# TThuraya/multimodal-PL

Hardware: AMD Instinct MI355X
Metric: train voxels/sec at 96^3 patch, 1/2/4/8 MI355X; fwd+bwd step ms (higher is better)
Workload: dtype bf16; 1 GPU; unet3D_baseline([1,2,2,2,2],16,weight_std) fwd+EDiceLoss_partial+bwd+SGD; model=unet3D_baseline-16, global_batch=2, seq_len=884736, parallelism=dp1, world_size_seen=1, force_buckets=False

## Files before the change

multimodal-pl_amd/csrc/common.h:

```cpp
#pragma once
#include <hip/hip_runtime.h>
#include <hip/hip_bf16.h>
#include <stdint.h>
#include <algorithm>
#include <string>
#include <type_traits>

#include "../../include/u3d.h"

namespace u3d {

void set_error(const std::string& msg);
int fail(int code, const char* fmt, ...);
int check_launch(const char* what);

enum Opt : int {
  OPT_IGEMM_BN,
  OPT_IGEMM_NS,
  OPT_IGEMM_TARGET,
  OPT_IGEMM_AUTO,
  OPT_CONVG_CO32,
  OPT_CONVG_PERSIST,
  OPT_CONVG_BW8,
  OPT_RING_KR,
  OPT_RING_WGS,
  OPT_RING_SC,
  OPT_SMALL_WGS,
  OPT_GN_MAXBLK,
  OPT_HEAD_TR,
  OPT_STEM1,
  OPT_UP_BWD_BLK,
  OPT_WGRAD_BD,
  OPT_WB_WGS,
  OPT_WR_TILE16,
  OPT_WR_WGS,
  OPT_WB_S2CO64,
  OPT_IGEMM_BM,
  OPT_WSTD_ROW,
  OPT_UP_QUAD,
  OPT_LOSS_PAIR,
  OPT_HEAD_NB,
  OPT_HEAD_GN_NB,
  OPT_STEM_MFMA,
  OPT_WB_S2BD,
  OPT_COUNT
};
int opt(Opt o);

#define U3D_REQUIRE(cond, ...)                                  \
  do {                                                          \
    if (!(cond)) return ::u3d::fail(U3D_EINVAL, __VA_ARGS__);   \
  } while (0)
#define U3D_HIP(expr)                                                               \
  do {                                                                              \
    hipError_t e_ = (expr);                                                         \
    if (e_ != hipSuccess)                                                           \
      return ::u3d::fail(U3D_EHIP, "%s: %s", #expr, hipGetErrorString(e_));         \
  } while (0)

template <int I, int N, typename F>
__device__ __forceinline__ void static_for(F&& f) {
  if constexpr (I < N) {
    f(std::integral_constant<int, I>{});
    static_for<I + 1, N>(f);
  }
}

typedef uint16_t bf16;

__device__ __forceinline__ float to_f(float v) { return v; }
__device__ __forceinline__ float to_f(bf16 v) { return __uint_as_float(((uint32_t)v) << 16); }

template <typename T> __device__ __forceinline__ T from_f(float v);
template <> __device__ __forceinline__ float from_f<float>(float v) { return v; }
template <> __device__ __forceinline__ bf16 from_f<bf16>(float v) {
  __hip_bfloat16 h = __float2bfloat16(v);
  return *reinterpret_cast<bf16*>(&h);
}

typedef __attribute__((ext_vector_type(4))) float f32x4;
typedef __attribute__((ext_vector_type(16))) float f32x16;
typedef __attribute__((ext_vector_type(8))) short s16x8;
typedef __attribute__((ext_vector_type(4))) uint32_t u32x4;

typedef __attribute__((ext_vector_type(2))) float f32x2;
typedef __attribute__((ext_vector_type(2))) __bf16 bf16x2_t;
typedef __attribute__((ext_vector_type(2))) short s16x2;

__device__ __forceinline__ uint32_t pack_bf16x2(float a, float b) {
  return __builtin_bit_cast(uint32_t, __builtin_convertvector((f32x2){a, b}, bf16x2_t));
}
__device__ __forceinline__ uint32_t relu_bf16x2(uint32_t u) {
  return __builtin_bit_cast(uint32_t, __builtin_elementwise_max(__builtin_bit_cast(s16x2, u), (s16x2){0, 0}));
}

template <int CTRL>
__device__ __forceinline__ float dpp_mov(float x) {
// ... 199 lines not shown
  *reinterpret_cast<u32x4*>(p) = r;
}

template <typename T, int N>
__device__ __forceinline__ void loadv(const T* p, float (&v)[N]) {
  if constexpr (N * sizeof(T) == 16) {
    load16<T>(p, v);
  } else {
#pragma unroll
    for (int i = 0; i < N; ++i) v[i] = to_f(p[i]);
  }
}
template <typename T, int N>
__device__ __forceinline__ void storev(T* p, const float (&v)[N]) {
  if constexpr (N * sizeof(T) == 16) {
    store16<T>(p, v);
  } else {
#pragma unroll
    for (int i = 0; i < N; ++i) p[i] = from_f<T>(v[i]);
  }
}

__device__ __forceinline__ u32x4 gn_relu8(u32x4 v, const f32x2 (&sc)[4], const f32x2 (&sh)[4]) {
  u32x4 o;
#pragma unroll
  for (int e = 0; e < 4; ++e) {
    const float f0 = fmaf(__uint_as_float(v[e] << 16), sc[e][0], sh[e][0]);
    const float f1 = fmaf(__uint_as_float(v[e] & 0xffff0000u), sc[e][1], sh[e][1]);
    o[e] = relu_bf16x2(pack_bf16x2(f0, f1));
  }
  return o;
}

__device__ __forceinline__ void gn_coef8(const float* __restrict__ st, const float* __restrict__ gamma,
                                         const float* __restrict__ beta, int groups, int cin, int n, int c0,
                                         f32x2 (&sc)[4], f32x2 (&sh)[4]) {
  const int cpg = cin / groups;
  const auto srs = __builtin_amdgcn_make_buffer_rsrc((void*)st, 0, 0x7FFFFFFF, 0x00020000);
  const auto grs = __builtin_amdgcn_make_buffer_rsrc((void*)gamma, 0, 0x7FFFFFFF, 0x00020000);
  const auto brs = __builtin_amdgcn_make_buffer_rsrc((void*)beta, 0, 0x7FFFFFFF, 0x00020000);
  asm volatile("" : "+v"(c0));
#pragma unroll
  for (int e = 0; e < 8; ++e) {
    const int c = min(c0 + e, cin - 1), gg = c / cpg;
    const int so = (n * groups + gg) * 8;
    const float mean = __builtin_bit_cast(float, __builtin_amdgcn_raw_buffer_load_b32(srs, so, 0, 0));
    const float rstd = __builtin_bit_cast(float, __builtin_amdgcn_raw_buffer_load_b32(srs, so + 4, 0, 0));
    const float s = rstd * __builtin_bit_cast(float, __builtin_amdgcn_raw_buffer_load_b32(grs, c * 4, 0, 0));
    sc[e >> 1][e & 1] = s;
    sh[e >> 1][e & 1] = __builtin_bit_cast(float, __builtin_amdgcn_raw_buffer_load_b32(brs, c * 4, 0, 0)) - mean * s;
  }
}

__device__ __forceinline__ float wave_sum(float v) {
#pragma unroll
  for (int o = 32; o > 0; o >>= 1) v += __shfl_xor(v, o, 64);
  return v;
}
__device__ __forceinline__ double wave_sum(double v) {
#pragma unroll
  for (int o = 32; o > 0; o >>= 1) v += __shfl_xor(v, o, 64);
  return v;
}

struct TileSplit {
  int tx, ty, split;
};
__device__ __forceinline__ TileSplit xcd_tile_split(int L, int gx, int gy, int total) {
  const int nt = gx * gy;
  const int q = total >> 3, rr = total & 7, xcd = L & 7, loc = L >> 3;
  const int N = (xcd < rr ? xcd * (q + 1) : rr * (q + 1) + (xcd - rr) * q) + loc;
  const int tile = N % nt;
  return TileSplit{tile % gx, tile / gx, N / nt};
}
__device__ __forceinline__ TileSplit xcd_tile_split() {
  return xcd_tile_split(blockIdx.x + gridDim.x * (blockIdx.y + gridDim.y * blockIdx.z), gridDim.x, gridDim.y,
                        gridDim.x * gridDim.y * gridDim.z);
}

__host__ __device__ inline int cdiv(long long a, long long b) { return (int)((a + b - 1) / b); }
__host__ __device__ inline int round_up(int a, int b) { return (a + b - 1) / b * b; }
inline bool fits_buffer_offsets(long long bytes) { return bytes < (1LL << 31) - 64; }

}
```

multimodal-pl_amd/csrc/conv.hip:

```cpp
#include <algorithm>
#include <cstdlib>

#include "common.h"

namespace u3d {

constexpr int BK = 32;
constexpr int NTHR = 256;

struct Geom {
  int cin, cout, cin_p, cout_p;
  int id, ih, iw;
  int od, oh, ow;
  int qd, qh, qw;
  int so, pod, poh, pow_;
  int si;
  int ntaps;
  int gn_groups;
  int nsamp, nsplit, kps;
  int mtiles, ntiles;
  float* slab;
  int tap_w[27];
  signed char tap_d[27], tap_h[27], tap_x[27];
};

template <typename T> struct MfmaTraits;
template <> struct MfmaTraits<bf16> {
  static constexpr int NCH = BK * 2 / 16;
  __device__ static int swz(int r, int c) { return c ^ ((r >> 2) & 3); }
};
template <> struct MfmaTraits<float> {
  static constexpr int NCH = BK * 4 / 16;
  __device__ static int swz(int r, int c) { return c ^ (r & 7); }
};

typedef __attribute__((ext_vector_type(8))) __bf16 bf16x8;

template <typename T, int TM, int TN>
__device__ __forceinline__ void mfma_step(const char* As, const char* Bs, int arow0, int brow0, int lane,
                                          f32x16 (&acc)[TM][TN]) {
  using TR = MfmaTraits<T>;
  constexpr int ROWB = BK * sizeof(T);
  const int r = lane & 31, h = lane >> 5;
  if constexpr (sizeof(T) == 2) {
#pragma unroll
    for (int s = 0; s < 2; ++s) {
      bf16x8 a[TM], b[TN];
#pragma unroll
      for (int tm = 0; tm < TM; ++tm) {
        int row = arow0 + tm * 32 + r;
        a[tm] = *reinterpret_cast<const bf16x8*>(As + row * ROWB + TR::swz(row, 2 * s + h) * 16);
      }
#pragma unroll
      for (int tn = 0; tn < TN; ++tn) {
        int row = brow0 + tn * 32 + r;
        b[tn] = *reinterpret_cast<const bf16x8*>(Bs + row * ROWB + TR::swz(row, 2 * s + h) * 16);
      }
#pragma unroll
      for (int tm = 0; tm < TM; ++tm)
#pragma unroll
        for (int tn = 0; tn < TN; ++tn)
          acc[tm][tn] = __builtin_amdgcn_mfma_f32_32x32x16_bf16(a[tm], b[tn], acc[tm][tn], 0, 0, 0);
    }
  } else {
#pragma unroll
    for (int j = 0; j < 4; ++j) {
      f32x4 a[TM], b[TN];
#pragma unroll
      for (int tm = 0; tm < TM; ++tm) {
        int row = arow0 + tm * 32 + r;
        a[tm] = *reinterpret_cast<const f32x4*>(As + row * ROWB + TR::swz(row, 4 * h + j) * 16);
      }
#pragma unroll
      for (int tn = 0; tn < TN; ++tn) {
// ... 149 lines not shown
  const int kk0 = split * g.kps, kk1 = min(nk, kk0 + g.kps);
  __syncthreads();
  if (kk0 < kk1) {
    gload(kk0);
    swrite(kk0, 0);
  }
  __syncthreads();
  for (int kk = kk0; kk < kk1; ++kk) {
    const int cur = (kk - kk0) & 1;
    if (kk + 1 < kk1) gload(kk + 1);
    mfma_step<T, TM, TN>(As(cur), Bs(cur), arow0, brow0, lane, acc);
    if (kk + 1 < kk1) swrite(kk + 1, cur ^ 1);
    __syncthreads();
  }

  const int r = lane & 31, h = lane >> 5;
  const long long out_n = (long long)n * g.od * g.oh * g.ow;
#pragma unroll
  for (int tn = 0; tn < TN; ++tn) {
    const int co = bn0 + brow0 + tn * 32 + r;
    if (co >= g.cout) continue;
    const float bv = bias ? bias[co] : 0.f;
#pragma unroll
    for (int tm = 0; tm < TM; ++tm) {
#pragma unroll
      for (int i = 0; i < 16; ++i) {
        const int q = bm0 + arow0 + tm * 32 + (i & 3) + 8 * (i >> 2) + 4 * h;
        if (q >= Mq) continue;
        if (g.nsplit > 1) {
          g.slab[(((long long)split * g.nsamp + n) * Mq + q) * g.cout + co] = acc[tm][tn][i];
          continue;
        }
        long long ov;
        if (g.so == 1) {
          ov = q;
        } else {
          int qw_ = q % g.qw, t = q / g.qw;
          int qh_ = t % g.qh, qd_ = t / g.qh;
          ov = ((long long)(qd_ * g.so + g.pod) * g.oh + (qh_ * g.so + g.poh)) * g.ow + (qw_ * g.so + g.pow_);
        }
        const long long off = (out_n + ov) * g.cout + co;
        float v = acc[tm][tn][i] + bv;
        if (res) v += to_f(res[off]);
        y[off] = from_f<TO>(v);
      }
    }
  }
}

template <int KC>
__device__ __forceinline__ int kswz(int r, int c) {
  if constexpr (KC == 4) return c ^ ((r >> 2) & 3);
  else return c ^ ((r >> 1) & 7);
}

template <typename TO, int BM, int BN, int WM, int WN, int KC>
__global__ __launch_bounds__(NTHR) void igemm_bf16_kernel(const bf16* __restrict__ x, const bf16* __restrict__ wpk,
                                                          TO* __restrict__ y, const bf16* __restrict__ res,
                                                          const float* __restrict__ bias,
                                                          const float* __restrict__ gstat,
                                                          const float* __restrict__ gamma,
                                                          const float* __restrict__ beta, Geom g) {
#ifndef U3D_IGEMM_D4
#define U3D_IGEMM_D4 3
#endif
#ifndef U3D_IGEMM_D8
#define U3D_IGEMM_D8 2
#endif
  constexpr int NCH = KC, ROWB = KC * 16, BKC = KC * 8, D = KC == 4 ? U3D_IGEMM_D4 : U3D_IGEMM_D8;
  constexpr int A_LOADS = BM * NCH / NTHR;
  constexpr int B_CH = BN * NCH;
  constexpr int B_LOADS = (B_CH + NTHR - 1) / NTHR;
  constexpr int TM = BM / WM / 32, TN = BN / WN / 32;
  static_assert(A_LOADS >= 1 && WM * WN == 4, "tile");

  __shared__ __attribute__((aligned(16))) char smem[2 * (BM + BN) * ROWB + 2 * 256 * 4 + 27 * 24];
  float* gsc = reinterpret_cast<float*>(smem + 2 * (BM + BN) * ROWB);
  float* gsh = gsc + 256;
  int* taps = reinterpret_cast<int*>(gsh + 256);
  int* tdhw = taps + 27 * 2;
  if (threadIdx.x < g.ntaps) {
    const int td = g.tap_d[threadIdx.x], th = g.tap_h[threadIdx.x], tx = g.tap_x[threadIdx.x];
    taps[threadIdx.x * 2] = (td * g.ih + th) * g.iw + tx;
    taps[threadIdx.x * 2 + 1] = g.tap_w[threadIdx.x];
    tdhw[threadIdx.x * 4] = td;
    tdhw[threadIdx.x * 4 + 1] = th;
    tdhw[threadIdx.x * 4 + 2] = tx;
  }
  __syncthreads();
  auto As = [&](int b) -> char* { return smem + b * (BM * ROWB); };
  auto Bs = [&](int b) -> char* { return smem + 2 * BM * ROWB + b * (BN * ROWB); };

  const int tid = threadIdx.x, lane = tid & 63, wave = tid >> 6;
  int wi;
  {
    const int nwg = gridDim.x, q8 = nwg >> 3, r8 = nwg & 7, xcd = blockIdx.x & 7, loc = blockIdx.x >> 3;
    wi = (xcd < r8 ? xcd * (q8 + 1) : r8 * (q8 + 1) + (xcd - r8) * q8) + loc;
  }
  const int tiles = g.mtiles * g.ntiles * g.nsamp;
  const int split = wi / tiles, trem = wi - split * tiles;
  const int n = trem / (g.mtiles * g.ntiles), mn = trem - n * (g.mtiles * g.ntiles);
  const int bm0 = (mn % g.mtiles) * BM, bn0 = (mn / g.mtiles) * BN;
  const int Mq = g.qd * g.qh * g.qw;
  const bool has_gn = gstat != nullptr;
  if (has_gn) build_gn_table(gsc, gsh, g.cin, g.gn_groups, gstat, gamma, beta, n);
  const bf16* xn = x + (long long)n * g.id * g.ih * g.iw * g.cin;

  int a_row[A_LOADS], a_ch[A_LOADS], a_base[A_LOADS];
  unsigned a_mask[A_LOADS];
#pragma unroll
  for (int i = 0; i < A_LOADS; ++i) {
    const int id = tid + i * NTHR;
    a_row[i] = id / NCH;
    a_ch[i] = id % NCH;
    const int q = bm0 + a_row[i];
    unsigned m = 0;
    int base = 0;
    if (q < Mq) {
      const int qw_ = q % g.qw, t = q / g.qw;
      const int bd = (t / g.qh) * g.si, bh = (t % g.qh) * g.si, bw = qw_ * g.si;
      base = (bd * g.ih + bh) * g.iw + bw;
      for (int tt = 0; tt < g.ntaps; ++tt) {
        const int zd = bd + tdhw[tt * 4], zh = bh + tdhw[tt * 4 + 1], zw = bw + tdhw[tt * 4 + 2];
        if ((unsigned)zd < (unsigned)g.id && (unsigned)zh < (unsigned)g.ih && (unsigned)zw < (unsigned)g.iw)
          m |= 1u << tt;
      }
    }
    a_base[i] = base;
    a_mask[i] = m;
  }
  const int nchunks = g.cin_p / BKC;
  const int nk = g.ntaps * nchunks;

  u32x4 ra[D][A_LOADS], rb[D][B_LOADS];
  unsigned am[D];
  auto gload = [&](int kk, int slot) {
    const int t = kk / nchunks, c0 = (kk - t * nchunks) * BKC;
    const int delta = taps[t * 2];
    unsigned m = 0;
#pragma unroll
    for (int i = 0; i < A_LOADS; ++i) {
      const int c = c0 + a_ch[i] * 8;
      const bool ok = ((a_mask[i] >> t) & 1u) && c < g.cin;
      const int off = ok ? (a_base[i] + delta) * g.cin + c : 0;
      ra[slot][i] = *reinterpret_cast<const u32x4*>(xn + off);
      m |= ok ? 1u << i : 0u;
    }
    am[slot] = m;
    const bf16* wt = wpk + (long long)taps[t * 2 + 1] * g.cout_p * g.cin_p;
#pragma unroll
    for (int i = 0; i < B_LOADS; ++i) {
      const int id = min(tid + i * NTHR, B_CH - 1);
      const int row = id / NCH, ch = id % NCH, co = min(bn0 + row, g.cout_p - 1);
      rb[slot][i] = *reinterpret_cast<const u32x4*>(wt + co * g.cin_p + c0 + ch * 8);
    }
  };
  auto swrite = [&](int kk, int slot, int buf) {
    const int t = kk / nchunks, c0 = (kk - t * nchunks) * BKC;
#pragma unroll
    for (int i = 0; i < A_LOADS; ++i) {
      u32x4 v = ra[slot][i];
      const bool ok = (am[slot] >> i) & 1u;
      if (!ok) v = u32x4{0u, 0u, 0u, 0u};
      if (has_gn && ok) {
        const int c = c0 + a_ch[i] * 8;
        f32x2 sc[4], sh[4];
#pragma unroll
        for (int e = 0; e < 4; ++e) {
          sc[e] = f32x2{gsc[c + 2 * e], gsc[c + 2 * e + 1]};
          sh[e] = f32x2{gsh[c + 2 * e], gsh[c + 2 * e + 1]};
        }
        v = gn_relu8(v, sc, sh);
      }
      *reinterpret_cast<u32x4*>(As(buf) + a_row[i] * ROWB + kswz<KC>(a_row[i], a_ch[i]) * 16) = v;
    }
#pragma unroll
    for (int i = 0; i < B_LOADS; ++i) {
      const int id = tid + i * NTHR;
      if (B_CH % NTHR == 0 || id < B_CH) {
        const int row = id / NCH, ch = id % NCH;
        u32x4 v = rb[slot][i];
        if (bn0 + row >= g.cout_p) v = u32x4{0u, 0u, 0u, 0u};
        *reinterpret_cast<u32x4*>(Bs(buf) + row * ROWB + kswz<KC>(row, ch) * 16) = v;
      }
    }
  };

  const int wr = wave / WN, wc = wave % WN;
  const int arow0 = wr * (BM / WM), brow0 = wc * (BN / WN);
  f32x16 acc[TM][TN];
  auto stage_mfma = [&](const char* Ab, const char* Bb) {
    const int r = lane & 31, h = lane >> 5;
#pragma unroll
    for (int s = 0; s < KC / 2; ++s) {
      bf16x8 av[TM], bv[TN];
#pragma unroll
      for (int tm = 0; tm < TM; ++tm) {
        const int row = arow0 + tm * 32 + r;
        av[tm] = *reinterpret_cast<const bf16x8*>(Ab + row * ROWB + kswz<KC>(row, 2 * s + h) * 16);
      }
#pragma unroll
      for (int tn = 0; tn < TN; ++tn) {
        const int row = brow0 + tn * 32 + r;
        bv[tn] = *reinterpret_cast<const bf16x8*>(Bb + row * ROWB + kswz<KC>(row, 2 * s + h) * 16);
      }
#pragma unroll
      for (int tm = 0; tm < TM; ++tm)
#pragma unroll
        for (int tn = 0; tn < TN; ++tn)
          acc[tm][tn] = __builtin_amdgcn_mfma_f32_32x32x16_bf16(av[tm], bv[tn], acc[tm][tn], 0, 0, 0);
    }
  };
#pragma unroll
  for (int tm = 0; tm < TM; ++tm)
#pragma unroll
    for (int tn = 0; tn < TN; ++tn)
#pragma unroll
      for (int e = 0; e < 16; ++e) acc[tm][tn][e] = 0.f;

  const int kk0 = split * g.kps, kk1 = min(nk, kk0 + g.kps);
  __syncthreads();
  if (kk0 < kk1) {
#pragma unroll
    for (int j = 0; j < D; ++j) gload(min(kk0 + j, kk1 - 1), j);
    swrite(kk0, 0, 0);
  }
  __syncthreads();
  int kk = kk0;
  for (; kk + D < kk1; kk += D) {
#pragma unroll
    for (int j = 0; j < D; ++j) {
      gload(min(kk + j + D, kk1 - 1), j);
      const int buf = (kk + j - kk0) & 1;
      stage_mfma(As(buf), Bs(buf));
      swrite(kk + j + 1, (j + 1) % D, buf ^ 1);
      __syncthreads();
    }
  }
#pragma unroll
  for (int j = 0; j < D; ++j) {
    if (kk + j < kk1) {
      const int buf = (kk + j - kk0) & 1;
      stage_mfma(As(buf), Bs(buf));
      if (kk + j + 1 < kk1) swrite(kk + j + 1, (j + 1) % D, buf ^ 1);
      __syncthreads();
    }
  }

  const int r = lane & 31, h = lane >> 5;
  const long long out_n = (long long)n * g.od * g.oh * g.ow;
#pragma unroll
  for (int tn = 0; tn < TN; ++tn) {
    const int co = bn0 + brow0 + tn * 32 + r;
    if (co >= g.cout) continue;
    const float bv = bias ? bias[co] : 0.f;
#pragma unroll
    for (int tm = 0; tm < TM; ++tm) {
#pragma unroll
      for (int i = 0; i < 16; ++i) {
        const int q = bm0 + arow0 + tm * 32 + (i & 3) + 8 * (i >> 2) + 4 * h;
        if (q >= Mq) continue;
        if (g.nsplit > 1) {
          g.slab[(((long long)split * g.nsamp + n) * Mq + q) * g.cout + co] = acc[tm][tn][i];
          continue;
        }
        long long ov;
        if (g.so == 1) {
          ov = q;
        } else {
          const int qw_ = q % g.qw, t = q / g.qw;
          const int qh_ = t % g.qh, qd_ = t / g.qh;
          ov = ((long long)(qd_ * g.so + g.pod) * g.oh + (qh_ * g.so + g.poh)) * g.ow + (qw_ * g.so + g.pow_);
        }
        const long long off = (out_n + ov) * g.cout + co;
        float v = acc[tm][tn][i] + bv;
        if (res) v += to_f(res[off]);
        y[off] = from_f<TO>(v);
      }
    }
  }
}

template <typename T>
__global__ __launch_bounds__(NTHR) void wgrad_kernel(const T* __restrict__ dy, const T* __restrict__ x,
                                                     const float* __restrict__ gstat, const float* __restrict__ gamma,
                                                     const float* __restrict__ beta, float* __restrict__ part,
                                                     Geom g, int n_samples, long long vox_per_split) {
  constexpr int KV = 32;
  constexpr int VEC = 16 / sizeof(T);
  constexpr int CH = 32 / VEC;
  constexpr int NLD = KV * CH;
  constexpr int LOADS = (NLD + NTHR - 1) / NTHR;
  constexpr int TILE_B = 32 * 32 * sizeof(T);
  static_assert(NLD <= NTHR * LOADS, "wgrad tile");
  using TR = MfmaTraits<T>;

  __shared__ __attribute__((aligned(16))) char smem[5 * TILE_B];
  __shared__ float gsc[256], gsh[256];

  const int tid = threadIdx.x, lane = tid & 63, wave = tid >> 6;
  const int ci0 = blockIdx.x * 32, co0 = blockIdx.y * 32;
  const int tgroups = (g.ntaps + 3) / 4;
  const int tg = blockIdx.z % tgroups, split = blockIdx.z / tgroups;
  const int t0 = tg * 4;
  const int ntl = min(4, g.ntaps - t0);
  const int Mq = g.qd * g.qh * g.qw;
  const long long Mtot = (long long)n_samples * Mq;
  const long long v0 = split * vox_per_split;
  const long long v1 = min(Mtot, v0 + vox_per_split);
  const bool has_gn = gstat != nullptr;

  f32x16 acc;
#pragma unroll
  for (int e = 0; e < 16; ++e) acc[e] = 0.f;

  int cur_gn_n = -1;
  float rdy[LOADS][VEC], rx[4][LOADS][VEC];

  for (long long vb = v0; vb < v1; vb += KV) {
    if (has_gn) {
      int nfirst = (int)(vb / Mq);
      int nlast = (int)(min(v1, vb + KV) - 1) / Mq;
      if (nfirst != cur_gn_n || nlast != nfirst) {
        __syncthreads();
        build_gn_table(gsc, gsh, g.cin, g.gn_groups, gstat, gamma, beta, nfirst);
        cur_gn_n = nfirst;
        __syncthreads();
      }
    }
#pragma unroll
    for (int i = 0; i < LOADS; ++i) {
      int id = tid + i * NTHR;
      if (NLD % NTHR != 0 && id >= NLD) continue;
// ... 114 lines not shown
      p[(long long)co * g.cin_p + ci0 + r] = acc[i];
    }
  }
}

static void fill_taps(Geom& g, int ksize, bool transpose) {
  int p = ksize / 2, t = 0;
  for (int a = 0; a < ksize; ++a)
    for (int b = 0; b < ksize; ++b)
      for (int c = 0; c < ksize; ++c) {
        g.tap_w[t] = (a * ksize + b) * ksize + c;
        g.tap_d[t] = transpose ? p - a : a - p;
        g.tap_h[t] = transpose ? p - b : b - p;
        g.tap_x[t] = transpose ? p - c : c - p;
        ++t;
      }
  g.ntaps = t;
}

template <typename T, typename TO>
__global__ __launch_bounds__(256) void splitk_reduce_kernel(Geom g, const T* __restrict__ res,
                                                           const float* __restrict__ bias, TO* __restrict__ y) {
  const int Mq = g.qd * g.qh * g.qw;
  const long long per = (long long)g.nsamp * Mq * g.cout;
  for (long long i = blockIdx.x * 256LL + threadIdx.x; i < per; i += (long long)gridDim.x * 256) {
    const int co = (int)(i % g.cout);
    const long long nq = i / g.cout;
    const int q = (int)(nq % Mq), n = (int)(nq / Mq);
    float v = bias ? bias[co] : 0.f;
    for (int s = 0; s < g.nsplit; ++s) v += g.slab[s * per + i];
    long long ov;
    if (g.so == 1) {
      ov = q;
    } else {
      int qw_ = q % g.qw, t = q / g.qw;
      int qh_ = t % g.qh, qd_ = t / g.qh;
      ov = ((long long)(qd_ * g.so + g.pod) * g.oh + (qh_ * g.so + g.poh)) * g.ow + (qw_ * g.so + g.pow_);
    }
    const long long off = ((long long)n * g.od * g.oh * g.ow + ov) * g.cout + co;
    if (res) v += to_f(res[off]);
    y[off] = from_f<TO>(v);
  }
}

template <typename TO>
struct IgemmArgs {
  const bf16 *x, *wpk;
  TO* y;
  const bf16* res;
  const float *bias, *st, *ga, *be;
  hipStream_t s;
};

template <typename TO, int BM, int BN, int WM, int WN>
static void launch_igemm_bf16(const Geom& g, const IgemmArgs<TO>& a) {
  const dim3 grid(g.mtiles * g.ntiles * g.nsamp * g.nsplit);
  if (g.cin_p % 64 == 0)
    hipLaunchKernelGGL((igemm_bf16_kernel<TO, BM, BN, WM, WN, 8>), grid, dim3(NTHR), 0, a.s, a.x, a.wpk, a.y, a.res,
                       a.bias, a.st, a.ga, a.be, g);
  else
    hipLaunchKernelGGL((igemm_bf16_kernel<TO, BM, BN, WM, WN, 4>), grid, dim3(NTHR), 0, a.s, a.x, a.wpk, a.y, a.res,
                       a.bias, a.st, a.ga, a.be, g);
}

template <typename T, typename TO>
static int launch_igemm(Geom g, int n, const T* x, const T* wpk, TO* y, const T* res, const float* bias,
                        const float* st, const float* ga, const float* be, float* ws, long long ws_bytes,
                        hipStream_t s) {
  const int Mq = g.qd * g.qh * g.qw;
  if (Mq <= 0) return U3D_OK;
  const int env_bn = opt(OPT_IGEMM_BN), env_ns = opt(OPT_IGEMM_NS), env_target = opt(OPT_IGEMM_TARGET);
  int BN = g.cout_p <= 32 ? 32 : (sizeof(T) == 2 && g.cout_p >= 128) ? 128 : 64;
  const bool auto_bn = opt(OPT_IGEMM_AUTO) != 0;
  if (sizeof(T) == 2 && auto_bn) {
    auto ntile = [&](int bn) { return (long long)cdiv(Mq, 128) * cdiv(g.cout, bn) * n; };
    if (BN > 32 && ntile(BN) < 256) BN /= 2;
    if (BN > 32 && ntile(BN) < 64) BN /= 2;
  }
  if (env_bn && sizeof(T) == 2 && env_bn <= g.cout_p) BN = env_bn;
  const long long tiles = (long long)cdiv(Mq, 128) * cdiv(g.cout, BN) * n;
  const int nk = g.ntaps * (g.cin_p / BK);
  int ns = 1;
  if (ws && tiles < 256 && nk >= 8) {
    ns = (int)std::min<long long>(nk / 4, (env_target + tiles - 1) / tiles);
    if (env_ns > 0) ns = std::min(env_ns, nk);
    if (sizeof(T) == 2 && ns > 8) ns = ns / 8 * 8;
    const long long slab1 = (long long)n * Mq * g.cout * 4;
    while (ns > 1 && ns * slab1 > ws_bytes) --ns;
  }
  g.nsamp = n;
  g.nsplit = ns;
  g.kps = (nk + ns - 1) / ns;
  g.slab = ns > 1 ? ws : nullptr;
  if constexpr (sizeof(T) == 2) {
    const int env_bm = opt(OPT_IGEMM_BM);
    const bool bm256 = BN == 64 && ns == 1 && (env_bm == 256 || (env_bm == 0 && (long long)cdiv(Mq, 256) *
                                                                                 cdiv(g.cout, 64) * n >= 256));
    g.mtiles = cdiv(Mq, bm256 ? 256 : 128);
    g.ntiles = cdiv(g.cout, BN);
    if (g.cin_p % 64 == 0) {
      g.kps = (g.ntaps * (g.cin_p / 64) + ns - 1) / ns;
      g.nsplit = ns = std::min(ns, g.ntaps * (g.cin_p / 64));
    }
    const IgemmArgs<TO> a{x, wpk, y, res, bias, st, ga, be, s};
    if (BN == 32) launch_igemm_bf16<TO, 128, 32, 4, 1>(g, a);
    else if (BN == 64 && bm256) launch_igemm_bf16<TO, 256, 64, 2, 2>(g, a);
    else if (BN == 64) launch_igemm_bf16<TO, 128, 64, 2, 2>(g, a);
    else launch_igemm_bf16<TO, 128, 128, 2, 2>(g, a);
  } else if (BN == 32) {
    dim3 grid(cdiv(Mq, 128), cdiv(g.cout, 32), n * ns);
    hipLaunchKernelGGL((igemm_kernel<T, TO, 128, 32, 4, 1>), grid, dim3(NTHR), 0, s, x, wpk, y, res, bias, st, ga,
                       be, g);
  } else {
    dim3 grid(cdiv(Mq, 128), cdiv(g.cout, 64), n * ns);
    hipLaunchKernelGGL((igemm_kernel<T, TO, 128, 64, 2, 2>), grid, dim3(NTHR), 0, s, x, wpk, y, res, bias, st, ga,
                       be, g);
  }
  int rc = check_launch("igemm_kernel");
  if (rc || ns == 1) return rc;
  const long long per = (long long)n * Mq * g.cout;
  const int nb = (int)std::min<long long>(4096, (per + 255) / 256);
  hipLaunchKernelGGL((splitk_reduce_kernel<T, TO>), dim3(nb), dim3(256), 0, s, g, res, bias, y);
  return check_launch("splitk_reduce_kernel");
}

static int out_dim(int d, int k, int s) { return (d + 2 * (k / 2) - k) / s + 1; }

static Geom igemm_geom(int cin, int cout, int d, int h, int w, int ksize, int stride) {
  Geom g{};
  g.cin = cin; g.cout = cout; g.cin_p = round_up(cin, 32); g.cout_p = round_up(cout, 32);
  g.id = d; g.ih = h; g.iw = w;
  g.od = g.qd = out_dim(d, ksize, stride);
  g.oh = g.qh = out_dim(h, ksize, stride);
  g.ow = g.qw = out_dim(w, ksize, stride);
  g.so = 1; g.si = stride;
  return g;
}

}

using namespace u3d;

extern "C" int u3d_conv_fwd(int dtype, const void* x, int n, int cin, int d, int h, int w, const void* wpk, int cout,
                            int ksize, int stride, const float* gn_stats, const float* gn_gamma, const float* gn_beta,
                            int gn_groups, const void* residual, const float* bias, void* y, int y_f32,
                            float* ws, long long ws_bytes, u3d_stream_t stream) {
  U3D_REQUIRE(dtype == U3D_F32 || dtype == U3D_BF16, "conv_fwd: bad dtype %d", dtype);
  U3D_REQUIRE(ksize == 1 || ksize == 3, "conv_fwd: ksize %d unsupported", ksize);
  U3D_REQUIRE(stride == 1 || stride == 2, "conv_fwd: stride %d unsupported", stride);
  U3D_REQUIRE(cin % 8 == 0 && cin <= 4096, "conv_fwd: cin %d must be a multiple of 8 (stem: u3d_stem_fwd)", cin);
  U3D_REQUIRE(cout >= 1 && n >= 1 && d >= 1 && h >= 1 && w >= 1, "conv_fwd: bad shape");
  U3D_REQUIRE(x && wpk && y, "conv_fwd: null pointer");
  U3D_REQUIRE(!gn_stats || (gn_gamma && gn_beta && gn_groups > 0 && cin % gn_groups == 0 && cin <= 256),
              "conv_fwd: bad GroupNorm prologue (groups %d, cin %d)", gn_groups, cin);
  U3D_REQUIRE(!(y_f32 && residual), "conv_fwd: residual with fp32 output unsupported");
  Geom g = igemm_geom(cin, cout, d, h, w, ksize, stride);
  g.gn_groups = gn_groups;
  fill_taps(g, ksize, false);
  hipStream_t s = (hipStream_t)stream;
  if (dtype == U3D_BF16) {
    if (y_f32)
// ... 108 lines not shown
```

multimodal-pl_amd/csrc/runtime.cpp:

```cpp
#include <hip/hip_runtime.h>

#include <atomic>
#include <cstdarg>
#include <cstdio>
#include <cstdlib>
#include <cstring>
#include <mutex>
#include <string>

#include "common.h"

namespace u3d {

static thread_local std::string g_last_error;

void set_error(const std::string& msg) { g_last_error = msg; }

int fail(int code, const char* fmt, ...) {
  char buf[1024];
  va_list ap;
  va_start(ap, fmt);
  vsnprintf(buf, sizeof(buf), fmt, ap);
  va_end(ap);
  g_last_error = buf;
  return code;
}

int check_launch(const char* what) {
  hipError_t e = hipGetLastError();
  if (e != hipSuccess) return fail(U3D_EHIP, "%s launch: %s", what, hipGetErrorString(e));
  return U3D_OK;
}

namespace {
struct OptDef {
  const char* name;
  int dflt;
};
constexpr OptDef kOpts[OPT_COUNT] = {
    {"IGEMM_BN", 0},       {"IGEMM_NS", 0},     {"IGEMM_TARGET", 512}, {"IGEMM_AUTO", 1}, {"CONVG_CO32", -1},
    {"CONVG_PERSIST", 1},  {"CONVG_BW8", -1},   {"RING_KR", -1},       {"RING_WGS", 256}, {"RING_SC", 0},
    {"SMALL_WGS", 256},    {"GN_MAXBLK", 256},  {"HEAD_TR", 1},        {"STEM1", 1},      {"UP_BWD_BLK", -1},
    {"WGRAD_BD", 3},       {"WB_WGS", 256},     {"WR_TILE16", 0},      {"WR_WGS", 256},     {"WB_S2CO64", 1},
    {"IGEMM_BM", 128}, {"WSTD_ROW", 1}, {"UP_QUAD", 1}, {"LOSS_PAIR", 1},
    {"HEAD_NB", 768},  {"HEAD_GN_NB", 512}, {"STEM_MFMA", 1}, {"WB_S2BD", 3},
};
std::atomic<int> g_opt[OPT_COUNT];
std::once_flag g_opt_once;

void opt_init() {
  std::call_once(g_opt_once, [] {
    for (int i = 0; i < OPT_COUNT; ++i) {
      const std::string env = std::string("U3D_") + kOpts[i].name;
      const char* e = getenv(env.c_str());
      g_opt[i].store(e ? atoi(e) : kOpts[i].dflt);
    }
  });
}
}

int opt(Opt o) {
  opt_init();
  return g_opt[o].load(std::memory_order_relaxed);
}

}

extern "C" int u3d_set_option(const char* name, int value) {
  u3d::opt_init();
  for (int i = 0; i < u3d::OPT_COUNT; ++i)
    if (name && strcmp(name, u3d::kOpts[i].name) == 0) {
      u3d::g_opt[i].store(value);
      return U3D_OK;
    }
  return u3d::fail(U3D_EINVAL, "u3d_set_option: unknown option '%s'", name ? name : "(null)");
}

extern "C" int u3d_get_option(const char* name, int* value) {
  u3d::opt_init();
  for (int i = 0; i < u3d::OPT_COUNT; ++i)
    if (name && value && strcmp(name, u3d::kOpts[i].name) == 0) {
      *value = u3d::g_opt[i].load();
      return U3D_OK;
    }
  return u3d::fail(U3D_EINVAL, "u3d_get_option: unknown option '%s'", name ? name : "(null)");
}

extern "C" const char* u3d_last_error(void) { return u3d::g_last_error.c_str(); }
extern "C" int u3d_abi_version(void) { return 1; }
```

multimodal-pl_amd/csrc/wgrad_ring.hip:

```cpp
#include "wgrad_ring_body.h"

namespace u3d {
namespace {
U3D_STAMP_BUFFER(wr_stamps, 4096, u3d_diag_wgrad_stamps)
}

template <bool GN, int PH = 16, int PW = 16>
__global__ __launch_bounds__(WR_NT, 1) void wgrad_ring_kernel(const bf16* __restrict__ dy, const bf16* __restrict__ x,
                                                             const float* __restrict__ gstat,
                                                             const float* __restrict__ gamma,
                                                             const float* __restrict__ beta, float* __restrict__ part,
                                                             WRGeom g) {
  __shared__ __attribute__((aligned(16))) char lds[wr_lds_bytes<GN, PH, PW>()];
  wgrad_ring_body<GN, PH, PW>(lds, (int)(blockIdx.x + gridDim.x * (blockIdx.y + gridDim.y * blockIdx.z)),
                              (int)(gridDim.x * gridDim.y * gridDim.z), (int)gridDim.x, (int)gridDim.y, dy, x, gstat, gamma,
                              beta, part, g, wr_stamps);
}


constexpr int WD_HROWS = 352;
constexpr int WD_HP = WD_HROWS * 32;
constexpr int WD_SLOT = 2 * WD_HP;
constexpr int WD_DHP = 256 * 32;
constexpr int WD_DSLOT = 2 * WD_DHP;
constexpr int WD_NXS = 5, WD_NDS = 3;
#ifndef U3D_WD_LA
#define U3D_WD_LA 1
#endif
constexpr int WD_LA = U3D_WD_LA;
constexpr int WD_LDS = WD_NXS * WD_SLOT + WD_NDS * WD_DSLOT + 1024;
static_assert(WD_LDS <= 160 * 1024, "LDS");

typedef __attribute__((ext_vector_type(4))) unsigned u32x4s;
__device__ __forceinline__ u32x4s buf_desc(const void* base, int bytes) {
  const unsigned long long a = (unsigned long long)base;
  return u32x4s{(unsigned)a, (unsigned)(a >> 32) & 0xffffu, (unsigned)bytes, 0x00020000u};
}
#pragma clang diagnostic push
#pragma clang diagnostic ignored "-Winline-asm"
__device__ __forceinline__ void dma16(const u32x4s& rsrc, const char* lds_dst, unsigned off) {
  const unsigned m0 = __builtin_amdgcn_readfirstlane((unsigned)(uintptr_t)(__attribute__((address_space(3))) char*)lds_dst);
  asm volatile("s_mov_b32 m0, %1\n\ts_nop 0\n\tbuffer_load_dwordx4 %0, %2, 0 offen lds" : : "v"(off), "s"(m0),
               "s"(rsrc) : "memory", "m0");
}
#pragma clang diagnostic pop

template <bool GN>
__global__ __launch_bounds__(WR_NT, 1) void wgrad_ring_dma_kernel(const bf16* __restrict__ dy, const bf16* __restrict__ x,
                                                                 const float* __restrict__ gstat,
                                                                 const float* __restrict__ gamma,
                                                                 const float* __restrict__ beta,
                                                                 float* __restrict__ part, WRGeom g) {
  constexpr int HW = 18, NR = 324, PW = 16, KS2 = 8;
  __shared__ __attribute__((aligned(16))) char lds[WD_LDS];
  char* const ring = lds;
  char* const dyr = lds + WD_NXS * WD_SLOT;
  char* const junk = dyr + WD_NDS * WD_DSLOT;
  const int tid = threadIdx.x, lane = tid & 63, wave = __builtin_amdgcn_readfirstlane(tid >> 6);
  const int hf = wave >> 2, wv = wave & 3;
  const int cofs = 16 * hf + 8 * (lane & 1);
  const TileSplit ts = xcd_tile_split();
  const int ci0 = ts.tx * 32, co0 = ts.ty * 32, split = ts.split;
  WRWalk walk{};
  walk.o_next = (long long)split * g.per;
  walk.o_end = min(g.planes, walk.o_next + g.per);
  walk.done = false;
  walk.zin = 1;
  walk.zlast = 0;
  const u32x4s xrs = buf_desc(x, (int)g.xbytes), yrs = buf_desc(dy, (int)g.ybytes);
  f32x2 sc[4], sh[4];
  int gn_n = -1;
  const bool cok = ci0 + cofs < g.cin, dok = co0 + cofs < g.cout;

  int xlo[3], ylo[2], xhh[3], xhw[3];
#pragma unroll
  for (int j = 0; j < 3; ++j) {
    const int row = 32 * (wv + 4 * j) + (lane >> 1);
    xhh[j] = row / HW;
    xhw[j] = row % HW;
    xlo[j] = ((xhh[j] * g.w + xhw[j]) * g.cin + ci0 + cofs) * 2;
  }
#pragma unroll
  for (int j = 0; j < 2; ++j) {
    const int v = 32 * (wv + 4 * j) + (lane >> 1);
    ylo[j] = (((v >> 4) * g.w + (v & 15)) * g.cout + co0 + cofs) * 2;
  }
  unsigned xin = 0, yin = 0;
  int col_h0 = -1, col_w0 = -1;
  auto column = [&](const WRPlane& p) {
    if (p.valid && (p.h0 != col_h0 || p.w0 != col_w0)) {
      col_h0 = p.h0;
      col_w0 = p.w0;
      xin = yin = 0;
#pragma unroll
      for (int j = 0; j < 3; ++j) {
        const int i = wv + 4 * j, row = 32 * i + (lane >> 1);
        const bool ok = cok && i < 11 && row < NR && (unsigned)(p.h0 - 1 + xhh[j]) < (unsigned)g.h &&
                        (unsigned)(p.w0 - 1 + xhw[j]) < (unsigned)g.w;
// ... 246 lines not shown
```

Before: 324.7 million voxels/s.

## Add direct-to-LDS buffer-load pipelined variant of bf16 implicit-GEMM conv kernel

Adds a new implicit-GEMM conv kernel that loads A and B tiles with buffer_load ... lds straight into shared memory, bypassing registers, using a 2- or 3-stage ring. Stage issue is interleaved with the MFMA k-steps, and out-of-range taps go to an out-of-bounds offset instead of being guarded by branches. A heuristic picks the stage depth from LDS occupancy. The path is on by default for convs without a fused GroupNorm input whose cin is a multiple of 8. It shares its helpers with the wgrad ring kernel, and it risks lower occupancy from the larger LDS footprint.

```diff
diff --git a/multimodal-pl_amd/csrc/common.h b/multimodal-pl_amd/csrc/common.h
--- a/multimodal-pl_amd/csrc/common.h
+++ b/multimodal-pl_amd/csrc/common.h
@@ -43,6 +43,7 @@
   OPT_HEAD_GN_NB,
   OPT_STEM_MFMA,
   OPT_WB_S2BD,
+  OPT_IGEMM_DMA,
   OPT_COUNT
 };
 int opt(Opt o);
@@ -348,6 +349,26 @@
   }
 }
 
+typedef __attribute__((ext_vector_type(4))) unsigned u32x4s;
+__device__ __forceinline__ u32x4s buf_desc(const void* base, int bytes) {
+  const unsigned long long a = (unsigned long long)base;
+  return u32x4s{(unsigned)a, (unsigned)(a >> 32) & 0xffffu, (unsigned)bytes, 0x00020000u};
+}
+#pragma clang diagnostic push
+#pragma clang diagnostic ignored "-Winline-asm"
+__device__ __forceinline__ unsigned lds_addr(const char* p) {
+  return (unsigned)(uintptr_t)(__attribute__((address_space(3))) char*)p;
+}
+__device__ __forceinline__ void dma16_at(const u32x4s& rsrc, unsigned lds_dst, unsigned off) {
+  const unsigned m0 = __builtin_amdgcn_readfirstlane(lds_dst);
+  asm volatile("s_mov_b32 m0, %1\n\ts_nop 0\n\tbuffer_load_dwordx4 %0, %2, 0 offen lds" : : "v"(off), "s"(m0),
+               "s"(rsrc) : "memory", "m0");
+}
+__device__ __forceinline__ void dma16(const u32x4s& rsrc, const char* lds_dst, unsigned off) {
+  dma16_at(rsrc, lds_addr(lds_dst), off);
+}
+#pragma clang diagnostic pop
+
 __device__ __forceinline__ float wave_sum(float v) {
 #pragma unroll
   for (int o = 32; o > 0; o >>= 1) v += __shfl_xor(v, o, 64);
diff --git a/multimodal-pl_amd/csrc/conv.hip b/multimodal-pl_amd/csrc/conv.hip
--- a/multimodal-pl_amd/csrc/conv.hip
+++ b/multimodal-pl_amd/csrc/conv.hip
@@ -20,6 +20,7 @@
   int nsamp, nsplit, kps;
   int mtiles, ntiles;
   float* slab;
+  int xbytes, wbytes;
   int tap_w[27];
   signed char tap_d[27], tap_h[27], tap_x[27];
 };
@@ -275,6 +276,85 @@
 __device__ __forceinline__ int kswz(int r, int c) {
   if constexpr (KC == 4) return c ^ ((r >> 2) & 3);
   else return c ^ ((r >> 1) & 7);
+}
+
+struct IgemmTile {
+  int split, n, bm0, bn0;
+};
+template <int BM, int BN>
+__device__ __forceinline__ IgemmTile igemm_tile(const Geom& g) {
+  const int nwg = gridDim.x, q8 = nwg >> 3, r8 = nwg & 7, xcd = blockIdx.x & 7, loc = blockIdx.x >> 3;
+  const int wi = (xcd < r8 ? xcd * (q8 + 1) : r8 * (q8 + 1) + (xcd - r8) * q8) + loc;
+  const int tiles = g.mtiles * g.ntiles * g.nsamp;
+  const int split = wi / tiles, trem = wi - split * tiles;
+  const int n = trem / (g.mtiles * g.ntiles), mn = trem - n * (g.mtiles * g.ntiles);
+  return IgemmTile{split, n, (mn % g.mtiles) * BM, (mn / g.mtiles) * BN};
+}
+
+template <int KC, int TM, int TN, typename Side>
+__device__ __forceinline__ void igemm_stage_mfma(const char* Ab, const char* Bb, int arow0, int brow0, int lane,
+                                                 f32x16 (&acc)[TM][TN], Side&& side) {
+  constexpr int ROWB = KC * 16;
+  const int r = lane & 31, h = lane >> 5;
+  static_for<0, KC / 2>([&](auto sc) {
+    constexpr int s = decltype(sc)::value;
+    bf16x8 av[TM], bv[TN];
+#pragma unroll
+    for (int tm = 0; tm < TM; ++tm) {
+      const int row = arow0 + tm * 32 + r;
+      av[tm] = *reinterpret_cast<const bf16x8*>(Ab + row * ROWB + kswz<KC>(row, 2 * s + h) * 16);
+    }
+#pragma unroll
+    for (int tn = 0; tn < TN; ++tn) {
+      const int row = brow0 + tn * 32 + r;
+      bv[tn] = *reinterpret_cast<const bf16x8*>(Bb + row * ROWB + kswz<KC>(row, 2 * s + h) * 16);
+    }
+    side(sc);
+#pragma unroll
+    for (int tm = 0; tm < TM; ++tm)
+#pragma unroll
+      for (int tn = 0; tn < TN; ++tn)
+        acc[tm][tn] = __builtin_amdgcn_mfma_f32_32x32x16_bf16(av[tm], bv[tn], acc[tm][tn], 0, 0, 0);
+  });
+}
+
+template <typename TO, int TM, int TN>
+__device__ __forceinline__ void igemm_store(const Geom& g, const f32x16 (&acc)[TM][TN], int split, int n, int row0,
+                                            int col0, int lane, TO* __restrict__ y, const bf16* __restrict__ res,
+                                            const float* __restrict__ bias) {
+  const int Mq = g.qd * g.qh * g.qw;
+  const int r = lane & 31, h = lane >> 5;
+  const long long out_n = (long long)n * g.od * g.oh * g.ow;
+#pragma unroll
+  for (int tn = 0; tn < TN; ++tn) {
+    const int co = col0 + tn * 32 + r;
+    if (co >= g.cout) continue;
+    const float bv = bias ? bias[co] : 0.f;
+#pragma unroll
+    for (int tm = 0; tm < TM; ++tm) {
+#pragma unroll
+      for (int i = 0; i < 16; ++i) {
+        const int q = row0 + tm * 32 + (i & 3) + 8 * (i >> 2) + 4 * h;
+        if (q >= Mq) continue;
+        if (g.nsplit > 1) {
+          g.slab[(((long long)split * g.nsamp + n) * Mq + q) * g.cout + co] = acc[tm][tn][i];
+          continue;
+        }
+        long long ov;
+        if (g.so == 1) {
+          ov = q;
+        } else {
+          const int qw_ = q % g.qw, t = q / g.qw;
+          const int qh_ = t % g.qh, qd_ = t / g.qh;
+          ov = ((long long)(qd_ * g.so + g.pod) * g.oh + (qh_ * g.so + g.poh)) * g.ow + (qw_ * g.so + g.pow_);
+        }
+        const long long off = (out_n + ov) * g.cout + co;
+        float v = acc[tm][tn][i] + bv;
+        if (res) v += to_f(res[off]);
+        y[off] = from_f<TO>(v);
+      }
+    }
+  }
 }
 
 template <typename TO, int BM, int BN, int WM, int WN, int KC>
@@ -315,15 +395,8 @@
   auto Bs = [&](int b) -> char* { return smem + 2 * BM * ROWB + b * (BN * ROWB); };
 
   const int tid = threadIdx.x, lane = tid & 63, wave = tid >> 6;
-  int wi;
-  {
-    const int nwg = gridDim.x, q8 = nwg >> 3, r8 = nwg & 7, xcd = blockIdx.x & 7, loc = blockIdx.x >> 3;
-    wi = (xcd < r8 ? xcd * (q8 + 1) : r8 * (q8 + 1) + (xcd - r8) * q8) + loc;
-  }
-  const int tiles = g.mtiles * g.ntiles * g.nsamp;
-  const int split = wi / tiles, trem = wi - split * tiles;
-  const int n = trem / (g.mtiles * g.ntiles), mn = trem - n * (g.mtiles * g.ntiles);
-  const int bm0 = (mn % g.mtiles) * BM, bn0 = (mn / g.mtiles) * BN;
+  const IgemmTile tl = igemm_tile<BM, BN>(g);
+  const int split = tl.split, n = tl.n, bm0 = tl.bm0, bn0 = tl.bn0;
   const int Mq = g.qd * g.qh * g.qw;
   const bool has_gn = gstat != nullptr;
   if (has_gn) build_gn_table(gsc, gsh, g.cin, g.gn_groups, gstat, gamma, beta, n);
@@ -413,26 +486,7 @@
   const int arow0 = wr * (BM / WM), brow0 = wc * (BN / WN);
   f32x16 acc[TM][TN];
   auto stage_mfma = [&](const char* Ab, const char* Bb) {
-    const int r = lane & 31, h = lane >> 5;
-#pragma unroll
-    for (int s = 0; s < KC / 2; ++s) {
-      bf16x8 av[TM], bv[TN];
-#pragma unroll
-      for (int tm = 0; tm < TM; ++tm) {
-        const int row = arow0 + tm * 32 + r;
-        av[tm] = *reinterpret_cast<const bf16x8*>(Ab + row * ROWB + kswz<KC>(row, 2 * s + h) * 16);
-      }
-#pragma unroll
-      for (int tn = 0; tn < TN; ++tn) {
-        const int row = brow0 + tn * 32 + r;
-        bv[tn] = *reinterpret_cast<const bf16x8*>(Bb + row * ROWB + kswz<KC>(row, 2 * s + h) * 16);
-      }
-#pragma unroll
-      for (int tm = 0; tm < TM; ++tm)
-#pragma unroll
-        for (int tn = 0; tn < TN; ++tn)
-          acc[tm][tn] = __builtin_amdgcn_mfma_f32_32x32x16_bf16(av[tm], bv[tn], acc[tm][tn], 0, 0, 0);
-    }
+    igemm_stage_mfma<KC>(Ab, Bb, arow0, brow0, lane, acc, [](auto) {});
   };
 #pragma unroll
   for (int tm = 0; tm < TM; ++tm)
@@ -470,38 +524,146 @@
     }
   }
 
-  const int r = lane & 31, h = lane >> 5;
-  const long long out_n = (long long)n * g.od * g.oh * g.ow;
-#pragma unroll
-  for (int tn = 0; tn < TN; ++tn) {
-    const int co = bn0 + brow0 + tn * 32 + r;
-    if (co >= g.cout) continue;
-    const float bv = bias ? bias[co] : 0.f;
-#pragma unroll
-    for (int tm = 0; tm < TM; ++tm) {
-#pragma unroll
-      for (int i = 0; i < 16; ++i) {
-        const int q = bm0 + arow0 + tm * 32 + (i & 3) + 8 * (i >> 2) + 4 * h;
-        if (q >= Mq) continue;
-        if (g.nsplit > 1) {
-          g.slab[(((long long)split * g.nsamp + n) * Mq + q) * g.cout + co] = acc[tm][tn][i];
-          continue;
-        }
-        long long ov;
-        if (g.so == 1) {
-          ov = q;
-        } else {
-          const int qw_ = q % g.qw, t = q / g.qw;
-          const int qh_ = t % g.qh, qd_ = t / g.qh;
-          ov = ((long long)(qd_ * g.so + g.pod) * g.oh + (qh_ * g.so + g.poh)) * g.ow + (qw_ * g.so + g.pow_);
-        }
-        const long long off = (out_n + ov) * g.cout + co;
-        float v = acc[tm][tn][i] + bv;
-        if (res) v += to_f(res[off]);
-        y[off] = from_f<TO>(v);
-      }
-    }
-  }
+  igemm_store<TO>(g, acc, split, n, bm0 + arow0, bn0 + brow0, lane, y, res, bias);
+}
+
+constexpr int IGEMM_DMA_TABLES = 1024 + 27 * 24;
+constexpr int igemm_dma_lds(int BM, int BN, int KC, int S) { return S * (BM + BN) * KC * 16 + IGEMM_DMA_TABLES; }
+
+template <typename TO, int BM, int BN, int WM, int WN, int KC, int S>
+__global__ __launch_bounds__(NTHR) void igemm_bf16_dma_kernel(const bf16* __restrict__ x, const bf16* __restrict__ wpk,
+                                                              TO* __restrict__ y, const bf16* __restrict__ res,
+                                                              const float* __restrict__ bias, Geom g) {
+  constexpr int ROWB = KC * 16, BKC = KC * 8;
+  constexpr int RPI = 1024 / ROWB;
+  constexpr int A_N = BM / RPI, B_N = BN / RPI;
+  constexpr int A_I = A_N / 4, B_I = (B_N + 3) / 4, P = A_I + B_I;
+  constexpr int STAGE = (BM + BN) * ROWB;
+  constexpr int TM = BM / WM / 32, TN = BN / WN / 32;
+  constexpr unsigned OOR = 0xFFFFFFF0u;
+  static_assert(A_N % 4 == 0 && WM * WN == 4 && NTHR == 256 && S >= 2 && (S - 2) * P <= 63, "tile");
+  static_assert(igemm_dma_lds(BM, BN, KC, S) <= 160 * 1024, "LDS");
+
+  __shared__ __attribute__((aligned(16))) char smem[igemm_dma_lds(BM, BN, KC, S)];
+  char* const junk = smem + S * STAGE;
+  int* taps = reinterpret_cast<int*>(junk + 1024);
+  int* tdhw = taps + 27 * 2;
+  if (threadIdx.x < g.ntaps) {
+    const int td = g.tap_d[threadIdx.x], th = g.tap_h[threadIdx.x], tx = g.tap_x[threadIdx.x];
+    taps[threadIdx.x * 2] = (td * g.ih + th) * g.iw + tx;
+    taps[threadIdx.x * 2 + 1] = g.tap_w[threadIdx.x];
+    tdhw[threadIdx.x * 4] = td;
+    tdhw[threadIdx.x * 4 + 1] = th;
+    tdhw[threadIdx.x * 4 + 2] = tx;
+  }
+  __syncthreads();
+
+  const int tid = threadIdx.x, lane = tid & 63, wave = __builtin_amdgcn_readfirstlane(tid >> 6);
+  const IgemmTile tl = igemm_tile<BM, BN>(g);
+  const int split = tl.split, n = tl.n, bm0 = tl.bm0, bn0 = tl.bn0;
+  const int Mq = g.qd * g.qh * g.qw;
+  const u32x4s xrs = buf_desc(x + (long long)n * g.id * g.ih * g.iw * g.cin, g.xbytes);
+  const u32x4s wrs = buf_desc(wpk, g.wbytes);
+
+  const int lrow = lane / KC, lslot = lane % KC;
+  int a_base[A_I], a_coff[A_I], b_off[B_I];
+  unsigned a_mask[A_I];
+#pragma unroll
+  for (int j = 0; j < A_I; ++j) {
+    const int row = (wave + 4 * j) * RPI + lrow;
+    a_coff[j] = kswz<KC>(row, lslot) * 8;
+    const int q = bm0 + row;
+    unsigned m = 0;
+    int base = 0;
+    if (q < Mq) {
+      const int qw_ = q % g.qw, t = q / g.qw;
+      const int bd = (t / g.qh) * g.si, bh = (t % g.qh) * g.si, bw = qw_ * g.si;
+      base = (bd * g.ih + bh) * g.iw + bw;
+      for (int tt = 0; tt < g.ntaps; ++tt) {
+        const int zd = bd + tdhw[tt * 4], zh = bh + tdhw[tt * 4 + 1], zw = bw + tdhw[tt * 4 + 2];
+        if ((unsigned)zd < (unsigned)g.id && (unsigned)zh < (unsigned)g.ih && (unsigned)zw < (unsigned)g.iw)
+          m |= 1u << tt;
+      }
+    }
+    a_base[j] = base;
+    a_mask[j] = m;
+  }
+#pragma unroll
+  for (int j = 0; j < B_I; ++j) {
+    const int i = wave + 4 * j, row = i * RPI + lrow, co = bn0 + row;
+    b_off[j] = i < B_N && co < g.cout_p ? (co * g.cin_p + kswz<KC>(row, lslot) * 8) * 2 : -1;
+  }
+
+  const int nchunks = g.cin_p / BKC;
+  const int nk = g.ntaps * nchunks;
+  const int kk0 = split * g.kps, kk1 = min(nk, kk0 + g.kps), nst = kk1 - kk0;
+
+  int it = kk0 / nchunks, ic = kk0 - it * nchunks, ileft = nst;
+  int s_t = 0, s_c0 = 0, s_delta = 0, s_wb = 0;
+  bool s_live = false;
+  auto begin_stage = [&]() {
+    s_live = ileft > 0;
+    s_t = min(it, g.ntaps - 1);
+    s_c0 = ic * BKC;
+    s_delta = taps[s_t * 2];
+    s_wb = (taps[s_t * 2 + 1] * g.cout_p * g.cin_p + s_c0) * 2;
+    --ileft;
+    if (++ic == nchunks) {
+      ic = 0;
+      ++it;
+    }
+  };
+  const unsigned lds0 = lds_addr(smem), ljunk = lds_addr(junk);
+  auto piece = [&](int slot, auto pc) {
+    constexpr int p = decltype(pc)::value;
+    const unsigned sb = lds0 + slot * STAGE;
+    const unsigned live = s_live ? 1u : 0u;
+    if constexpr (p < A_I) {
+      const int c = s_c0 + a_coff[p];
+      const unsigned ok = (a_mask[p] >> s_t) & live & (c < g.cin ? 1u : 0u);
+      const unsigned off = (unsigned)(((a_base[p] + s_delta) * g.cin + c) * 2);
+      dma16_at(xrs, sb + (wave + 4 * p) * 1024, ok ? off : OOR);
+    } else {
+      constexpr int j = p - A_I;
+      const int i = wave + 4 * j;
+      const unsigned ok = live & (b_off[j] >= 0 ? 1u : 0u);
+      dma16_at(wrs, B_N % 4 == 0 || i < B_N ? sb + BM * ROWB + i * 1024 : ljunk, ok ? (unsigned)(s_wb + b_off[j]) : OOR);
+    }
+  };
+
+  const int wr = wave / WN, wc = wave % WN;
+  const int arow0 = wr * (BM / WM), brow0 = wc * (BN / WN);
+  f32x16 acc[TM][TN];
+#pragma unroll
+  for (int tm = 0; tm < TM; ++tm)
+#pragma unroll
+    for (int tn = 0; tn < TN; ++tn)
+#pragma unroll
+      for (int e = 0; e < 16; ++e) acc[tm][tn][e] = 0.f;
+
+  int islot = 0, rslot = 0;
+  for (int j = 0; j < S - 1; ++j) {
+    begin_stage();
+    static_for<0, P>([&](auto pc) { piece(islot, pc); });
+    islot = islot == S - 1 ? 0 : islot + 1;
+  }
+  for (int i = 0; i < nst; ++i) {
+    __builtin_amdgcn_sched_barrier(0);
+    asm volatile("s_waitcnt vmcnt(%0)\n\ts_waitcnt lgkmcnt(0)\n\ts_barrier" ::"n"((S - 2) * P) : "memory");
+    __builtin_amdgcn_sched_barrier(0);
+    begin_stage();
+    const char* const sb = smem + rslot * STAGE;
+    igemm_stage_mfma<KC>(sb, sb + BM * ROWB, arow0, brow0, lane, acc, [&](auto sc) {
+      static_for<0, (P - decltype(sc)::value + KC / 2 - 1) / (KC / 2)>([&](auto uc) {
+        piece(islot, std::integral_constant<int, decltype(sc)::value + decltype(uc)::value * (KC / 2)>{});
+      });
+    });
+    islot = islot == S - 1 ? 0 : islot + 1;
+    rslot = rslot == S - 1 ? 0 : rslot + 1;
+  }
+  asm volatile("s_waitcnt vmcnt(0)" ::: "memory");
+
+  igemm_store<TO>(g, acc, split, n, bm0 + arow0, bn0 + brow0, lane, y, res, bias);
 }
 
 template <typename T>
@@ -722,15 +884,40 @@
   hipStream_t s;
 };
 
+static bool igemm_dma_deep(int BM, int BN, int KC, long long grid) {
+#ifdef U3D_IGEMM_DMA_S
+  return U3D_IGEMM_DMA_S == 3;
+#endif
+  const int cap = (BM / 64) * (BN / 64) >= 4 ? 2 : 4;
+  auto rounds = [&](int S) {
+    const int per_cu = std::min(cap, 160 * 1024 / igemm_dma_lds(BM, BN, KC, S));
+    return per_cu > 0 ? cdiv(grid, 256LL * per_cu) : 1 << 30;
+  };
+  return rounds(3) <= rounds(2);
+}
+
+template <typename TO, int BM, int BN, int WM, int WN, int KC>
+static void launch_igemm_bf16_kc(const Geom& g, const IgemmArgs<TO>& a, bool dma) {
+  const dim3 grid(g.mtiles * g.ntiles * g.nsamp * g.nsplit);
+  if (!dma)
+    hipLaunchKernelGGL((igemm_bf16_kernel<TO, BM, BN, WM, WN, KC>), grid, dim3(NTHR), 0, a.s, a.x, a.wpk, a.y, a.res,
+                       a.bias, a.st, a.ga, a.be, g);
+  else if constexpr (igemm_dma_lds(BM, BN, KC, 3) <= 160 * 1024) {
+    if (igemm_dma_deep(BM, BN, KC, grid.x))
+      hipLaunchKernelGGL((igemm_bf16_dma_kernel<TO, BM, BN, WM, WN, KC, 3>), grid, dim3(NTHR), 0, a.s, a.x, a.wpk, a.y,
+                         a.res, a.bias, g);
+    else
+      hipLaunchKernelGGL((igemm_bf16_dma_kernel<TO, BM, BN, WM, WN, KC, 2>), grid, dim3(NTHR), 0, a.s, a.x, a.wpk, a.y,
+                         a.res, a.bias, g);
+  } else
+    hipLaunchKernelGGL((igemm_bf16_dma_kernel<TO, BM, BN, WM, WN, KC, 2>), grid, dim3(NTHR), 0, a.s, a.x, a.wpk, a.y,
+                       a.res, a.bias, g);
+}
+
 template <typename TO, int BM, int BN, int WM, int WN>
-static void launch_igemm_bf16(const Geom& g, const IgemmArgs<TO>& a) {
-  const dim3 grid(g.mtiles * g.ntiles * g.nsamp * g.nsplit);
-  if (g.cin_p % 64 == 0)
-    hipLaunchKernelGGL((igemm_bf16_kernel<TO, BM, BN, WM, WN, 8>), grid, dim3(NTHR), 0, a.s, a.x, a.wpk, a.y, a.res,
-                       a.bias, a.st, a.ga, a.be, g);
-  else
-    hipLaunchKernelGGL((igemm_bf16_kernel<TO, BM, BN, WM, WN, 4>), grid, dim3(NTHR), 0, a.s, a.x, a.wpk, a.y, a.res,
-                       a.bias, a.st, a.ga, a.be, g);
+static void launch_igemm_bf16(const Geom& g, const IgemmArgs<TO>& a, bool dma) {
+  if (g.cin_p % 64 == 0) launch_igemm_bf16_kc<TO, BM, BN, WM, WN, 8>(g, a, dma);
+  else launch_igemm_bf16_kc<TO, BM, BN, WM, WN, 4>(g, a, dma);
 }
 
 template <typename T, typename TO>
@@ -773,10 +960,16 @@
       g.nsplit = ns = std::min(ns, g.ntaps * (g.cin_p / 64));
     }
     const IgemmArgs<TO> a{x, wpk, y, res, bias, st, ga, be, s};
-    if (BN == 32) launch_igemm_bf16<TO, 128, 32, 4, 1>(g, a);
-    else if (BN == 64 && bm256) launch_igemm_bf16<TO, 256, 64, 2, 2>(g, a);
-    else if (BN == 64) launch_igemm_bf16<TO, 128, 64, 2, 2>(g, a);
-    else launch_igemm_bf16<TO, 128, 128, 2, 2>(g, a);
+    const long long xbytes = (long long)g.id * g.ih * g.iw * g.cin * 2;
+    const long long wbytes = (*std::max_element(g.tap_w, g.tap_w + g.ntaps) + 1LL) * g.cout_p * g.cin_p * 2;
+    const bool dma = opt(OPT_IGEMM_DMA) != 0 && !st && g.cin % 8 == 0 && fits_buffer_offsets(xbytes) &&
+                     fits_buffer_offsets(wbytes);
+    g.xbytes = (int)xbytes;
+    g.wbytes = (int)wbytes;
+    if (BN == 32) launch_igemm_bf16<TO, 128, 32, 4, 1>(g, a, dma);
+    else if (BN == 64 && bm256) launch_igemm_bf16<TO, 256, 64, 2, 2>(g, a, dma);
+    else if (BN == 64) launch_igemm_bf16<TO, 128, 64, 2, 2>(g, a, dma);
+    else launch_igemm_bf16<TO, 128, 128, 2, 2>(g, a, dma);
   } else if (BN == 32) {
     dim3 grid(cdiv(Mq, 128), cdiv(g.cout, 32), n * ns);
     hipLaunchKernelGGL((igemm_kernel<T, TO, 128, 32, 4, 1>), grid, dim3(NTHR), 0, s, x, wpk, y, res, bias, st, ga,
diff --git a/multimodal-pl_amd/csrc/runtime.cpp b/multimodal-pl_amd/csrc/runtime.cpp
--- a/multimodal-pl_amd/csrc/runtime.cpp
+++ b/multimodal-pl_amd/csrc/runtime.cpp
@@ -44,6 +44,7 @@
     {"WGRAD_BD", 3},       {"WB_WGS", 256},     {"WR_TILE16", 0},      {"WR_WGS", 256},     {"WB_S2CO64", 1},
     {"IGEMM_BM", 128}, {"WSTD_ROW", 1}, {"UP_QUAD", 1}, {"LOSS_PAIR", 1},
     {"HEAD_NB", 768},  {"HEAD_GN_NB", 512}, {"STEM_MFMA", 1}, {"WB_S2BD", 3},
+    {"IGEMM_DMA", 1},
 };
 std::atomic<int> g_opt[OPT_COUNT];
 std::once_flag g_opt_once;
diff --git a/multimodal-pl_amd/csrc/wgrad_ring.hip b/multimodal-pl_amd/csrc/wgrad_ring.hip
--- a/multimodal-pl_amd/csrc/wgrad_ring.hip
+++ b/multimodal-pl_amd/csrc/wgrad_ring.hip
@@ -30,20 +30,6 @@
 constexpr int WD_LA = U3D_WD_LA;
 constexpr int WD_LDS = WD_NXS * WD_SLOT + WD_NDS * WD_DSLOT + 1024;
 static_assert(WD_LDS <= 160 * 1024, "LDS");
-
-typedef __attribute__((ext_vector_type(4))) unsigned u32x4s;
-__device__ __forceinline__ u32x4s buf_desc(const void* base, int bytes) {
-  const unsigned long long a = (unsigned long long)base;
-  return u32x4s{(unsigned)a, (unsigned)(a >> 32) & 0xffffu, (unsigned)bytes, 0x00020000u};
-}
-#pragma clang diagnostic push
-#pragma clang diagnostic ignored "-Winline-asm"
-__device__ __forceinline__ void dma16(const u32x4s& rsrc, const char* lds_dst, unsigned off) {
-  const unsigned m0 = __builtin_amdgcn_readfirstlane((unsigned)(uintptr_t)(__attribute__((address_space(3))) char*)lds_dst);
-  asm volatile("s_mov_b32 m0, %1\n\ts_nop 0\n\tbuffer_load_dwordx4 %0, %2, 0 offen lds" : : "v"(off), "s"(m0),
-               "s"(rsrc) : "memory", "m0");
-}
-#pragma clang diagnostic pop
 
 template <bool GN>
 __global__ __launch_bounds__(WR_NT, 1) void wgrad_ring_dma_kernel(const bf16* __restrict__ dy, const bf16* __restrict__ x,
```

New measurement: 325.3 million voxels/s, median of 4. No clear change (+0.2%).
